# chacorp/latent-nerf-test

Hardware: AMD Instinct MI355X
Metric: latent-frames/sec (64x64x4, 128^3 grid), render forward+backward (higher is better)
Workload: dtype bf16

## Files before the change

### latent-nerf-test_amd/csrc/mlp_bf16.hip

```cpp
#include "common.h"
#include "mlp_shared.h"

namespace lnerf {

typedef __bf16 bf16x8 __attribute__((ext_vector_type(8)));
#define MFMA32(a, b, c) __builtin_amdgcn_mfma_f32_16x16x32_bf16((a), (b), (c), 0, 0, 0)

constexpr int F_W1A = 0;
constexpr int F_W2A = 4;
constexpr int F_W3A = 12;
constexpr int F_W3T = 14;
constexpr int F_W2T = 18;
constexpr int F_W1T = 26;
constexpr int F_FWD = 14, F_ALL = 30;

constexpr int RS = 68;

__device__ __forceinline__ int phi_of(int s, int q, int jj) { return 32 * s + 16 * (jj >> 2) + 4 * q + (jj & 3); }

__device__ __forceinline__ int frag_source(int e, int out_dim, int &idx) {
    const int f = e >> 9, l = (e >> 3) & 63, jj = e & 7;
    const int q = l >> 4, c = l & 15;
    if (f < F_W2A) {
        idx = (16 * (f - F_W1A) + c) * MLP_IN + 8 * q + jj;
        return 1;
    } else if (f < F_W3A) {
        const int mt = (f - F_W2A) >> 1, s = (f - F_W2A) & 1;
        idx = (16 * mt + c) * MLP_HID + phi_of(s, q, jj);
        return 2;
    } else if (f < F_W3T) {
        const int s = f - F_W3A;
        idx = c * MLP_HID + phi_of(s, q, jj);
        return c < out_dim ? 3 : 0;
    } else if (f < F_W2T) {
        const int mt = f - F_W3T, n = 4 * q + jj;
        idx = n * MLP_HID + 16 * mt + c;
        return (jj < 4 && n < out_dim) ? 3 : 0;
    } else if (f < F_W1T) {
        const int mt = (f - F_W2T) >> 1, s = (f - F_W2T) & 1;
        idx = phi_of(s, q, jj) * MLP_HID + 16 * mt + c;
        return 2;
    }
    const int mt = (f - F_W1T) >> 1, s = (f - F_W1T) & 1;
    idx = phi_of(s, q, jj) * MLP_IN + 16 * mt + c;
    return 1;
}

__device__ __forceinline__ void build_fragments(const MlpArgs &a, __bf16 *frag, int n_frag, int tid, int nthreads) {
    for (int e = tid; e < n_frag * 512; e += nthreads) {
        int idx;
        const int t = frag_source(e, a.out_dim, idx);
        const float v = t == 1 ? a.w1[idx] : t == 2 ? a.w2[idx] : t == 3 ? a.w3[idx] : 0.f;
        frag[e] = (__bf16)v;
    }
}

__global__ void __launch_bounds__(256) k_mlp_fragment_maps(int out_dim, int32_t *m1, int32_t *m2, int32_t *m3) {
    for (int e = blockIdx.x * 256 + threadIdx.x; e < F_ALL * 512; e += gridDim.x * 256) {
        int idx;
        const int t = frag_source(e, out_dim, idx);
        const int slot = (e >> 9) < F_W3T ? 0 : 1;
        int32_t *m = t == 1 ? m1 : t == 2 ? m2 : t == 3 ? m3 : nullptr;
        if (m) m[2 * idx + slot] = e;
    }
}

constexpr int F_SELX = 30;
constexpr int F_SEL3 = 32;
constexpr int F_SW = 33;
static_assert((size_t)F_SW * 1024 <= MLP_FRAG_BYTES, "fragment cache");
__device__ __forceinline__ void build_selectors(__bf16 *frag, int tid, int nthreads) {
    for (int e = tid; e < (F_SW - F_SELX) * 512; e += nthreads) {
        const int f = F_SELX + (e >> 9), l = (e >> 3) & 63, jj = e & 7;
        const int q = l >> 4, c = l & 15;
        const bool one = f < F_SEL3 ? (8 * q + jj == 16 * (f - F_SELX) + c) : (jj < 4 && 4 * q + jj == c);
        frag[F_SELX * 512 + e] = (__bf16)(one ? 1.0f : 0.0f);
    }
}
__global__ void __launch_bounds__(256) k_mlp_build_fragments(MlpArgs a, __bf16 *out, int n_frag) {
    build_fragments(a, out, n_frag < F_ALL ? n_frag : F_ALL, blockIdx.x * 256 + threadIdx.x, gridDim.x * 256);
    if (n_frag > F_ALL) build_selectors(out, blockIdx.x * 256 + threadIdx.x, gridDim.x * 256);
}
__device__ __forceinline__ void fetch_fragments(const MlpArgs &a, __bf16 *frag, int n_frag, int tid, int nthreads) {
    if (a.frag_global) {
        const uint4 *src = reinterpret_cast<const uint4 *>(a.frag_global);
        uint4 *dst = reinterpret_cast<uint4 *>(frag);
        for (int e = tid; e < n_frag * 64; e += nthreads) dst[e] = src[e];
    } else {
        build_fragments(a, frag, n_frag, tid, nthreads);
    }
}

__device__ __forceinline__ bf16x8 ld_frag(const __bf16 *frag, int f, int lane) {
    return *reinterpret_cast<const bf16x8 *>(frag + (f * 64 + lane) * 8);
}

__device__ __forceinline__ bf16x8 load_x(const MlpArgs &a, int64_t m, int q) {
    if (a.feat_bf16) {
        const char *f = reinterpret_cast<const char *>(a.feat);
        const uint32_t ls = (uint32_t)a.level_stride;
        uint32_t w[4];
#pragma unroll
        for (int k = 0; k < 4; ++k)
            w[k] = *reinterpret_cast<const uint32_t *>(f + (size_t)((((uint32_t)(4 * q + k)) * ls + (uint32_t)m) << 2));
        return *reinterpret_cast<bf16x8 *>(w);
    }
    bf16x8 x;
    const float2 *f = reinterpret_cast<const float2 *>(a.feat);
#pragma unroll
    for (int k = 0; k < 4; ++k) {
        const float2 v = f[(int64_t)(4 * q + k) * a.level_stride + m];
        x[2 * k] = (__bf16)v.x;
        x[2 * k + 1] = (__bf16)v.y;
    }
    return x;
}
__device__ __forceinline__ int64_t clamp_row(int64_t m, int64_t M) { return m < M ? m : (M > 0 ? M - 1 : 0); }

typedef short s16x2 __attribute__((ext_vector_type(2)));
typedef unsigned short u16x2 __attribute__((ext_vector_type(2)));
typedef __bf16 bf16x2 __attribute__((ext_vector_type(2)));

__device__ __forceinline__ uint32_t cvt_pk(float lo, float hi) {
    typedef float f32x2 __attribute__((ext_vector_type(2)));
    const f32x2 f = {lo, hi};
    return __builtin_bit_cast(uint32_t, __builtin_convertvector(f, bf16x2));
}
__device__ __forceinline__ uint32_t relu_pk(uint32_t v) {
    const s16x2 z = {0, 0};
    return __builtin_bit_cast(uint32_t, __builtin_elementwise_max(__builtin_bit_cast(s16x2, v), z));
}
__device__ __forceinline__ uint32_t live_pk(uint32_t act) {
    asm("" : "+v"(act));
    const s16x2 z = {0, 0};
    const s16x2 n = z - __builtin_bit_cast(s16x2, act);
    return __builtin_bit_cast(uint32_t, n >> 15);
}
union Pk8 {
    bf16x8 v;
    uint32_t u[4];
};
__device__ __forceinline__ bf16x8 pack_relu_pk(const f32x4 &lo, const f32x4 &hi) {
    Pk8 r;
    r.u[0] = relu_pk(cvt_pk(lo[0], lo[1]));
    r.u[1] = relu_pk(cvt_pk(lo[2], lo[3]));
    r.u[2] = relu_pk(cvt_pk(hi[0], hi[1]));
    r.u[3] = relu_pk(cvt_pk(hi[2], hi[3]));
    return r.v;
}
__device__ __forceinline__ bf16x8 pack_masked_pk(const f32x4 &lo, const f32x4 &hi, const bf16x8 &act) {
    Pk8 r, a;
    a.v = act;
    r.u[0] = cvt_pk(lo[0], lo[1]) & live_pk(a.u[0]);
    r.u[1] = cvt_pk(lo[2], lo[3]) & live_pk(a.u[1]);
    r.u[2] = cvt_pk(hi[0], hi[1]) & live_pk(a.u[2]);
    r.u[3] = cvt_pk(hi[2], hi[3]) & live_pk(a.u[3]);
    return r.v;
}
__device__ __forceinline__ bf16x8 pack_plain_pk(const f32x4 &lo, const f32x4 &hi) {
    Pk8 r;
    r.u[0] = cvt_pk(lo[0], lo[1]);
    r.u[1] = cvt_pk(lo[2], lo[3]);
    r.u[2] = cvt_pk(hi[0], hi[1]);
    r.u[3] = cvt_pk(hi[2], hi[3]);
    return r.v;
}
__device__ __forceinline__ float sum8(const bf16x8 &v, float acc) {
    Pk8 a;
    a.v = v;
    bf16x2 ones;
    ones[0] = (__bf16)1.0f;
    ones[1] = (__bf16)1.0f;
#pragma unroll
    for (int i = 0; i < 4; ++i) acc = __builtin_amdgcn_fdot2_f32_bf16(__builtin_bit_cast(bf16x2, a.u[i]), ones, acc, false);
    return acc;
}

__device__ __forceinline__ bf16x8 pack_relu(const f32x4 &lo, const f32x4 &hi) { return pack_relu_pk(lo, hi); }
__device__ __forceinline__ bf16x8 pack_masked(const f32x4 &lo, const f32x4 &hi, const bf16x8 &act) {
    return pack_masked_pk(lo, hi, act);
}

__device__ __forceinline__ f32x4 ld_bias4(const float *b, int base) {
    return (f32x4){b[base], b[base + 1], b[base + 2], b[base + 3]};
}

#ifdef LNERF_STAMPS
__device__ unsigned long long g_mlp_stamps[32];
struct Stamps {
    unsigned long long acc[16], prev;
    __device__ __forceinline__ void init() {
        for (int i = 0; i < 16; ++i) acc[i] = 0;
        prev = __builtin_amdgcn_s_memtime();
    }
    __device__ __forceinline__ void mark(int k) {
        const unsigned long long now = __builtin_amdgcn_s_memtime();
        acc[k] += now - prev;
        prev = now;
    }
    __device__ __forceinline__ void flush(int base) {
        if (threadIdx.x == 0)
            for (int i = 0; i < 16; ++i) atomicAdd(&g_mlp_stamps[base + i], acc[i]);
    }
};
#else
struct Stamps {
    __device__ __forceinline__ void init() {}
    __device__ __forceinline__ void mark(int) {}
    __device__ __forceinline__ void flush(int) {}
};
#endif

template <int T>
__device__ __forceinline__ void forward_hidden(const __bf16 *frag, const float *sB1, const float *sB2, int lane,
                                               const bf16x8 xB[T], bf16x8 h1B[2][T], bf16x8 h2B[2][T], Stamps &st) {
    const int q = lane >> 4;
    f32x4 acc[4][T];
#pragma unroll
    for (int mt = 0; mt < 4; ++mt) {
        const bf16x8 w = ld_frag(frag, F_W1A + mt, lane);
        const f32x4 b = ld_bias4(sB1, 16 * mt + 4 * q);
#pragma unroll
        for (int t = 0; t < T; ++t) acc[mt][t] = MFMA32(w, xB[t], b);
    }
#pragma unroll
    for (int s = 0; s < 2; ++s)
#pragma unroll
        for (int t = 0; t < T; ++t) h1B[s][t] = pack_relu(acc[2 * s][t], acc[2 * s + 1][t]);
    st.mark(1);
#pragma unroll
    for (int mt = 0; mt < 4; ++mt) {
        const f32x4 b = ld_bias4(sB2, 16 * mt + 4 * q);
#pragma unroll
        for (int t = 0; t < T; ++t) acc[mt][t] = b;
#pragma unroll
        for (int s = 0; s < 2; ++s) {
            const bf16x8 w = ld_frag(frag, F_W2A + 2 * mt + s, lane);
#pragma unroll
            for (int t = 0; t < T; ++t) acc[mt][t] = MFMA32(w, h1B[s][t], acc[mt][t]);
        }
    }
#pragma unroll
    for (int s = 0; s < 2; ++s)
#pragma unroll
        for (int t = 0; t < T; ++t) h2B[s][t] = pack_relu(acc[2 * s][t], acc[2 * s + 1][t]);
    st.mark(2);
}

template <int WPS>
__global__ void __launch_bounds__(256, WPS)
k_mlp_forward_bf16(MlpArgs a, float *__restrict__ sigmas, float *__restrict__ rgbs) {
    __shared__ __attribute__((aligned(16))) __bf16 frag[F_FWD * 512];
    __shared__ float sB1[MLP_HID], sB2[MLP_HID], sB3[16];
    int64_t M = a.m_host;
    if (a.m_dev) { const int64_t md = *a.m_dev; M = md < M ? md : M; }
    const int tid = threadIdx.x, lane = tid & 63, w = tid >> 6, q = lane >> 4, c = lane & 15;
    fetch_fragments(a, frag, F_FWD, tid, 256);
    if (tid < MLP_HID) { sB1[tid] = a.b1[tid]; sB2[tid] = a.b2[tid]; }
    if (tid < 16) sB3[tid] = tid < a.out_dim ? a.b3[tid] : 0.f;
    __syncthreads();
    const int nrgb = a.out_dim - 1;
    bf16x8 xB[2];
#pragma unroll
    for (int t = 0; t < 2; ++t) {
        const int64_t m = (int64_t)blockIdx.x * 128 + w * 32 + 16 * t + c;
        xB[t] = load_x(a, clamp_row(m, M), q);
    }
    Stamps st;
    st.init();
    for (int64_t tile = blockIdx.x; tile * 128 < M; tile += gridDim.x) {
        const int64_t m0 = tile * 128 + w * 32;
        bf16x8 xB_n[2], h1B[2][2], h2B[2][2];
#pragma unroll
        for (int t = 0; t < 2; ++t) {
            const int64_t m = m0 + (int64_t)gridDim.x * 128 + 16 * t + c;
            xB_n[t] = load_x(a, clamp_row(m, M), q);
        }
        st.mark(0);
        forward_hidden<2>(frag, sB1, sB2, lane, xB, h1B, h2B, st);
        const f32x4 b3 = ld_bias4(sB3, 4 * q);
        int lane3 = lane;
        asm("" : "+v"(lane3) : "s"((int)tile));
        const bf16x8 w3a = ld_frag(frag, F_W3A, lane3), w3b = ld_frag(frag, F_W3A + 1, lane3);
#pragma unroll
        for (int t = 0; t < 2; ++t) {
            f32x4 o = b3;
            o = MFMA32(w3a, h2B[0][t], o);
            o = MFMA32(w3b, h2B[1][t], o);
            const int64_t m = m0 + 16 * t + c;
            if (a.out_dim == 5) {
                const float r3 = __shfl_down(o[0], 16, 64);
                if (q == 0 && m < M) {
                    sigmas[m] = expf(o[0] + blob_of(a, m));
                    reinterpret_cast<float4 *>(rgbs)[m] = make_float4(o[1], o[2], o[3], r3);
                }
            } else if (m < M) {
#pragma unroll
                for (int r = 0; r < 4; ++r) {
                    const int n = 4 * q + r;
                    if (n == 0) sigmas[m] = expf(o[r] + blob_of(a, m));
                    else if (n < a.out_dim) rgbs[m * nrgb + (n - 1)] = o[r];
                }
            }
        }
        st.mark(3);
        xB[0] = xB_n[0];
        xB[1] = xB_n[1];
    }
    st.flush(0);
}

template <int T>
struct Upstream { float v[T][4], sg[T]; };

template <int T>
__device__ __forceinline__ Upstream<T> load_upstream(const MlpArgs &a, const float *__restrict__ sigmas,
                                                     const float *__restrict__ dsigmas, const float *__restrict__ drgbs,
                                                     int64_t m0, int64_t M, int q, int c) {
    const int nrgb = a.out_dim - 1;
    Upstream<T> u;
#pragma unroll
    for (int t = 0; t < T; ++t) {
        const int64_t m = m0 + 16 * t + c;
        const bool in = m < M;
        const int64_t mc = clamp_row(m, M);
        if (a.out_dim == 5) {
            const float ds = dsigmas[mc], sg = sigmas[mc];
            const float4 g = reinterpret_cast<const float4 *>(drgbs)[mc];
            const bool q0 = in && q == 0, q1 = in && q == 1;
            u.sg[t] = sg;
            u.v[t][0] = q0 ? ds : (q1 ? g.w : 0.f);
            u.v[t][1] = q0 ? g.x : 0.f;
            u.v[t][2] = q0 ? g.y : 0.f;
            u.v[t][3] = q0 ? g.z : 0.f;
        } else {
            u.sg[t] = 1.0f;
#pragma unroll
            for (int jj = 0; jj < 4; ++jj) u.v[t][jj] = 0.f;
            if (in && q == 0) { u.v[t][0] = dsigmas[m]; u.sg[t] = sigmas[m]; }
#pragma unroll
            for (int jj = 0; jj < 4; ++jj) {
                const int n = 4 * q + jj;
                if (in && n >= 1 && n < a.out_dim) u.v[t][jj] = drgbs[m * nrgb + (n - 1)];
            }
        }
    }
    return u;
}
__device__ __forceinline__ bool upstream_fragment(const float v[4], float sg, int q, bf16x8 &d3) {
    const float e15 = 3269017.3724721107f;
    const float v0 = q == 0 ? v[0] * fminf(sg, e15) : v[0];
    Pk8 d;
    d.u[0] = cvt_pk(v0, v[1]);
    d.u[1] = cvt_pk(v[2], v[3]);
    d.u[2] = 0u;
    d.u[3] = 0u;
    d3 = d.v;
    return (v0 != 0.f) || (v[1] != 0.f) || (v[2] != 0.f) || (v[3] != 0.f);
}

__device__ __forceinline__ void stage_pair(__bf16 *img, int row, int fa, int fb, const bf16x8 &v) {
    const uint4 u = *reinterpret_cast<const uint4 *>(&v);
    *reinterpret_cast<uint2 *>(img + row * RS + fa) = make_uint2(u.x, u.y);
    *reinterpret_cast<uint2 *>(img + row * RS + fb) = make_uint2(u.z, u.w);
}
__device__ __forceinline__ void stage_lo(__bf16 *img, int row, int fa, const bf16x8 &v) {
    const uint4 u = *reinterpret_cast<const uint4 *>(&v);
    *reinterpret_cast<uint2 *>(img + row * RS + fa) = make_uint2(u.x, u.y);
}

typedef short s16x4 __attribute__((ext_vector_type(4)));
__device__ __forceinline__ bf16x8 ld_tr(const __bf16 *img, int k, int f0, int lane) {
    typedef s16x4 __attribute__((address_space(3))) *lds_s16x4_p;
    const int g = lane >> 4, i = lane & 15;
    const __bf16 *p = img + (32 * k + 8 * g + (i >> 2)) * RS + f0 + 4 * (i & 3);
    union {
        struct { s16x4 lo, hi; } h;
        bf16x8 v;
    } u;
    u.h.lo = __builtin_amdgcn_ds_read_tr16_b64_v4i16((lds_s16x4_p)p);
    u.h.hi = __builtin_amdgcn_ds_read_tr16_b64_v4i16((lds_s16x4_p)(p + 4 * RS));
    return u.v;
}

template <int NW, int T>
__global__ void __launch_bounds__(NW * 64, (NW == 4 ? 2 : 4))
k_mlp_backward_bf16(MlpArgs a, const float *__restrict__ sigmas, const float *__restrict__ dsigmas,
                    const float *__restrict__ drgbs, float *__restrict__ dfeat, float *__restrict__ slabs) {
    constexpr int STEP = NW * 16 * T, KS = STEP / 32, NH = NW / 4, C2 = 4 / NH, C1 = 2 / NH;
    __shared__ __attribute__((aligned(16))) __bf16 frag[F_ALL * 512];
    __shared__ __attribute__((aligned(16))) __bf16 imgA[STEP * RS];
    __shared__ __attribute__((aligned(16))) __bf16 imgD[STEP * RS];
    __shared__ float sB1[MLP_HID], sB2[MLP_HID];
    int64_t M = a.m_host;
    if (a.m_dev) { const int64_t md = *a.m_dev; M = md < M ? md : M; }
    const int tid = threadIdx.x, lane = tid & 63, w = tid >> 6, q = lane >> 4, c = lane & 15;
    const int r = w & 3, h = w >> 2;
    fetch_fragments(a, frag, F_ALL, tid, NW * 64);
    if (tid < MLP_HID) { sB1[tid] = a.b1[tid]; sB2[tid] = a.b2[tid]; }
    __syncthreads();
    const f32x4 zero4 = (f32x4){0.f, 0.f, 0.f, 0.f};
    bf16x8 ones;
#pragma unroll
    for (int i = 0; i < 8; ++i) ones[i] = (__bf16)1.0f;

    f32x4 gW2[C2], gW1[C1], gB = zero4, gW3 = zero4;
    f32x4 gB1x = zero4, gB3 = zero4;
#pragma unroll
    for (int i = 0; i < C2; ++i) gW2[i] = zero4;
#pragma unroll
    for (int i = 0; i < C1; ++i) gW1[i] = zero4;
    const bool own_b2 = h == 0, own_b1 = h == NH - 1, own_w3 = h == 0, own_b3 = w == NW - 4;

    const int64_t wofs = (int64_t)w * 16 * T;
    Upstream<T> up = load_upstream<T>(a, sigmas, dsigmas, drgbs, (int64_t)blockIdx.x * STEP + wofs, M, q, c);
    bf16x8 xB[T];
#pragma unroll
    for (int t = 0; t < T; ++t) {
        const int64_t m = (int64_t)blockIdx.x * STEP + wofs + 16 * t + c;
        xB[t] = load_x(a, clamp_row(m, M), q);
    }
    Stamps st;
    st.init();
    for (int64_t tile = blockIdx.x; tile * STEP < M; tile += gridDim.x) {
        const int64_t m0 = tile * STEP + wofs, m1 = m0 + (int64_t)gridDim.x * STEP;
        const Upstream<T> up_c = up;
        bf16x8 xC[T], h1B[2][T], h2B[2][T], dzB[2][T], d3B[T];
#pragma unroll
        for (int t = 0; t < T; ++t) xC[t] = xB[t];
        up = load_upstream<T>(a, sigmas, dsigmas, drgbs, m1, M, q, c);
#pragma unroll
        for (int t = 0; t < T; ++t) xB[t] = load_x(a, clamp_row(m1 + 16 * t + c, M), q);
        bool live = false;
#pragma unroll
        for (int t = 0; t < T; ++t) live = upstream_fragment(up_c.v[t], up_c.sg[t], q, d3B[t]) || live;
        (void)live;
        st.mark(4);
        forward_hidden<T>(frag, sB1, sB2, lane, xC, h1B, h2B, st);
        __syncthreads();
        st.mark(5);
#pragma unroll
        for (int t = 0; t < T; ++t) {
            const int row = 16 * T * w + 16 * t + c;
#pragma unroll
            for (int s = 0; s < 2; ++s) stage_pair(imgA, row, 32 * s + 4 * q, 32 * s + 16 + 4 * q, h2B[s][t]);
            stage_lo(imgD, row, 4 * q, d3B[t]);
        }
        __syncthreads();
        st.mark(6);
        if (own_w3 || own_b3) {
#pragma unroll
            for (int k = 0; k < KS; ++k) {
                const bf16x8 dA = ld_tr(imgD, k, 0, lane);
                if (own_w3) gW3 = MFMA32(dA, ld_tr(imgA, k, 16 * r, lane), gW3);
                if (own_b3) gB3 = MFMA32(dA, ones, gB3);
            }
        }
        st.mark(7);
        {
            f32x4 acc[4][T];
#pragma unroll
            for (int mt = 0; mt < 4; ++mt) {
                const bf16x8 wf = ld_frag(frag, F_W3T + mt, lane);
#pragma unroll
                for (int t = 0; t < T; ++t) acc[mt][t] = MFMA32(wf, d3B[t], zero4);
            }
#pragma unroll
            for (int s = 0; s < 2; ++s)
#pragma unroll
                for (int t = 0; t < T; ++t) dzB[s][t] = pack_masked(acc[2 * s][t], acc[2 * s + 1][t], h2B[s][t]);
        }
        st.mark(8);
        __syncthreads();
#pragma unroll
        for (int t = 0; t < T; ++t) {
            const int row = 16 * T * w + 16 * t + c;
#pragma unroll
            for (int s = 0; s < 2; ++s) {
                stage_pair(imgA, row, 32 * s + 4 * q, 32 * s + 16 + 4 * q, h1B[s][t]);
                stage_pair(imgD, row, 32 * s + 4 * q, 32 * s + 16 + 4 * q, dzB[s][t]);
            }
        }
        __syncthreads();
        st.mark(9);
#pragma unroll
        for (int k = 0; k < KS; ++k) {
            const bf16x8 dA = ld_tr(imgD, k, 16 * r, lane);
#pragma unroll
            for (int i = 0; i < C2; ++i) gW2[i] = MFMA32(dA, ld_tr(imgA, k, 16 * (C2 * h + i), lane), gW2[i]);
            if (own_b2) gB = MFMA32(dA, ones, gB);
        }
        st.mark(10);
        {
            f32x4 acc[4][T];
#pragma unroll
            for (int mt = 0; mt < 4; ++mt) {
#pragma unroll
                for (int t = 0; t < T; ++t) acc[mt][t] = zero4;
#pragma unroll
                for (int s = 0; s < 2; ++s) {
                    const bf16x8 wf = ld_frag(frag, F_W2T + 2 * mt + s, lane);
#pragma unroll
                    for (int t = 0; t < T; ++t) acc[mt][t] = MFMA32(wf, dzB[s][t], acc[mt][t]);
                }
            }
#pragma unroll
            for (int s = 0; s < 2; ++s)
#pragma unroll
                for (int t = 0; t < T; ++t) dzB[s][t] = pack_masked(acc[2 * s][t], acc[2 * s + 1][t], h1B[s][t]);
        }
        st.mark(11);
        __syncthreads();
#pragma unroll
        for (int t = 0; t < T; ++t) {
            const int row = 16 * T * w + 16 * t + c;
            stage_pair(imgA, row, 8 * q, 8 * q + 4, xC[t]);
#pragma unroll
            for (int s = 0; s < 2; ++s) stage_pair(imgD, row, 32 * s + 4 * q, 32 * s + 16 + 4 * q, dzB[s][t]);
        }
        __syncthreads();
        st.mark(12);
#pragma unroll
        for (int k = 0; k < KS; ++k) {
            const bf16x8 dA = ld_tr(imgD, k, 16 * r, lane);
#pragma unroll
            for (int i = 0; i < C1; ++i) gW1[i] = MFMA32(dA, ld_tr(imgA, k, 16 * (C1 * h + i), lane), gW1[i]);
            if (own_b1) { if (NH == 1) gB1x = MFMA32(dA, ones, gB1x); else gB = MFMA32(dA, ones, gB); }
        }
        st.mark(13);
#pragma unroll
        for (int mt = 0; mt < 2; ++mt) {
            f32x4 ax[T];
#pragma unroll
            for (int t = 0; t < T; ++t) ax[t] = zero4;
#pragma unroll
            for (int s = 0; s < 2; ++s) {
                const bf16x8 wf = ld_frag(frag, F_W1T + 2 * mt + s, lane);
#pragma unroll
                for (int t = 0; t < T; ++t) ax[t] = MFMA32(wf, dzB[s][t], ax[t]);
            }
#pragma unroll
            for (int t = 0; t < T; ++t) {
                const int64_t m = m0 + 16 * t + c;
                if (m < M) {
                    const int lv = 8 * mt + 2 * q;
                    char *df = reinterpret_cast<char *>(dfeat);
                    const uint32_t ls = (uint32_t)a.level_stride, o0 = (((uint32_t)lv) * ls + (uint32_t)m) << 3;
                    *reinterpret_cast<float2 *>(df + (size_t)o0) = make_float2(ax[t][0], ax[t][1]);
                    *reinterpret_cast<float2 *>(df + (size_t)(o0 + (ls << 3))) = make_float2(ax[t][2], ax[t][3]);
                }
            }
        }
        st.mark(14);
    }

    st.flush(16);
    float *slab = slabs + (int64_t)blockIdx.x * MLP_SLAB;
#pragma unroll
    for (int rr = 0; rr < 4; ++rr) {
        const int o = 16 * r + 4 * q + rr;
#pragma unroll
        for (int i = 0; i < C2; ++i) slab[MLP_SL_W2 + o * MLP_HID + 16 * (C2 * h + i) + c] = gW2[i][rr];
#pragma unroll
        for (int i = 0; i < C1; ++i) slab[MLP_SL_W1 + o * MLP_IN + 16 * (C1 * h + i) + c] = gW1[i][rr];
        if (c == 0) {
            if (own_b2) slab[MLP_SL_B2 + o] = gB[rr];
            if (own_b1) slab[MLP_SL_B1 + o] = NH == 1 ? gB1x[rr] : gB[rr];
        }
        if (own_w3) slab[MLP_SL_W3 + (4 * q + rr) * MLP_HID + 16 * r + c] = gW3[rr];
        if (own_b3 && c == 0) slab[MLP_SL_B3 + 4 * q + rr] = gB3[rr];
    }
}

}

namespace lnerf {

#ifdef LNERF_STAMPS
int mlp_stamps_read(unsigned long long *out32) {
    unsigned long long z[32] = {0};
    if (hipMemcpyFromSymbol(out32, HIP_SYMBOL(g_mlp_stamps), sizeof(z)) != hipSuccess) return LNERF_ERR_HIP;
    if (hipMemcpyToSymbol(HIP_SYMBOL(g_mlp_stamps), z, sizeof(z)) != hipSuccess) return LNERF_ERR_HIP;
    return LNERF_OK;
}
#endif

int launch_mlp_fragment_maps(int out_dim, int32_t *m1, int32_t *m2, int32_t *m3, hipStream_t stream) {
    if (hipMemsetAsync(m1, 0xFF, (size_t)MLP_HID * MLP_IN * 2 * sizeof(int32_t), stream) != hipSuccess ||
        hipMemsetAsync(m2, 0xFF, (size_t)MLP_HID * MLP_HID * 2 * sizeof(int32_t), stream) != hipSuccess ||
        hipMemsetAsync(m3, 0xFF, (size_t)out_dim * MLP_HID * 2 * sizeof(int32_t), stream) != hipSuccess) {
        set_error("mlp_fragment_maps: hipMemsetAsync failed");
        return LNERF_ERR_HIP;
    }
    hipLaunchKernelGGL(k_mlp_fragment_maps, dim3(16), dim3(256), 0, stream, out_dim, m1, m2, m3);
    LNERF_CHECK_LAUNCH("mlp(fragment maps)");
    return LNERF_OK;
}

int launch_mlp_fragments_bf16(const MlpArgs &a, void *frag_out, bool backward_too, hipStream_t stream) {
    const int n = backward_too ? F_SW : F_FWD;
    hipLaunchKernelGGL(k_mlp_build_fragments, dim3((unsigned)(n * 2)), dim3(256), 0, stream, a, (__bf16 *)frag_out, n);
    LNERF_CHECK_LAUNCH("mlp(fragments)");
    return LNERF_OK;
}

int launch_mlp_forward_bf16(const MlpArgs &a, float *sigmas, float *rgbs, int blocks, int wps, hipStream_t stream) {
    if (wps >= 3) hipLaunchKernelGGL(k_mlp_forward_bf16<3>, dim3((unsigned)blocks), dim3(256), 0, stream, a, sigmas, rgbs);
    else hipLaunchKernelGGL(k_mlp_forward_bf16<2>, dim3((unsigned)blocks), dim3(256), 0, stream, a, sigmas, rgbs);
    LNERF_CHECK_LAUNCH("mlp_forward(bf16)");
    return LNERF_OK;
}

int launch_mlp_backward_bf16(const MlpArgs &a, const float *sigmas, const float *dsigmas, const float *drgbs,
                             float *dfeat, float *slabs, int blocks, hipStream_t stream) {
    hipLaunchKernelGGL((k_mlp_backward_bf16<4, 2>), dim3((unsigned)blocks), dim3(256), 0, stream, a, sigmas, dsigmas,
                       drgbs, dfeat, slabs);
    LNERF_CHECK_LAUNCH("mlp_backward(bf16)");
    return LNERF_OK;
}

}
```

### latent-nerf-test_amd/csrc/mlp_shared.h

```cpp
#pragma once
#include "common.h"

namespace lnerf {

typedef float f32x4 __attribute__((ext_vector_type(4)));

constexpr int MLP_IN = 32, MLP_HID = 64, MLP_OUTP = 16;

constexpr int MLP_SL_W1 = 0, MLP_SL_B1 = MLP_SL_W1 + MLP_HID * MLP_IN, MLP_SL_W2 = MLP_SL_B1 + MLP_HID,
              MLP_SL_B2 = MLP_SL_W2 + MLP_HID * MLP_HID, MLP_SL_W3 = MLP_SL_B2 + MLP_HID,
              MLP_SL_B3 = MLP_SL_W3 + MLP_OUTP * MLP_HID, MLP_SLAB = MLP_SL_B3 + MLP_OUTP;
constexpr int MLP_BWD_MAX_BLOCKS = 512;

struct MlpArgs {
    const void *feat;
    int feat_bf16;
    int64_t level_stride;
    const float *xyzs;
    const float *w1, *b1, *w2, *b2, *w3, *b3;
    int out_dim;
    float blob_scale, blob_denom;
    int64_t m_host;
    const int32_t *m_dev;
    const void *frag_global;
};
constexpr size_t MLP_FRAG_BYTES = LNERF_MLP_FRAGMENT_BYTES;

__device__ __forceinline__ float blob_of(const MlpArgs &a, int64_t m) {
    const float x = a.xyzs[m * 3], y = a.xyzs[m * 3 + 1], z = a.xyzs[m * 3 + 2];
    const float d2 = (x * x + y * y) + z * z;
    return a.blob_scale * expf(-d2 / a.blob_denom);
}

int launch_mlp_fragments_bf16(const MlpArgs &a, void *frag_out, bool backward_too, hipStream_t stream);
int launch_mlp_fragment_maps(int out_dim, int32_t *m1, int32_t *m2, int32_t *m3, hipStream_t stream);
int launch_mlp_forward_bf16(const MlpArgs &a, float *sigmas, float *rgbs, int blocks, int wps, hipStream_t stream);
int launch_mlp_backward_bf16(const MlpArgs &a, const float *sigmas, const float *dsigmas, const float *drgbs,
                             float *dfeat, float *slabs, int blocks, hipStream_t stream);

#ifdef LNERF_STAMPS
int mlp_stamps_read(unsigned long long *out32);
#endif

}
```

Baseline: 2663.

## Specialize MLP kernels on feature dtype/output width, prefetch positions, hold weights in registers

The forward and backward MLP kernels are now templated on whether features are bf16 and whether out_dim is 5, so runtime branches disappear. The forward kernel keeps the W1/W2 fragments and b1 bias in registers across tiles instead of re-reading them from LDS each tile. It also software-prefetches xyz positions for the blob term together with the next tile's features. Empty asm pins and sched_barriers force the prefetched loads to stay in flight across the compute, at the cost of higher VGPR pressure, which may reduce occupancy or cause spills.

```diff
diff --git a/latent-nerf-test_amd/csrc/mlp_bf16.hip b/latent-nerf-test_amd/csrc/mlp_bf16.hip
--- a/latent-nerf-test_amd/csrc/mlp_bf16.hip
+++ b/latent-nerf-test_amd/csrc/mlp_bf16.hip
@@ -95,8 +95,9 @@
     return *reinterpret_cast<const bf16x8 *>(frag + (f * 64 + lane) * 8);
 }
 
+template <bool FB16>
 __device__ __forceinline__ bf16x8 load_x(const MlpArgs &a, int64_t m, int q) {
-    if (a.feat_bf16) {
+    if (FB16) {
         const char *f = reinterpret_cast<const char *>(a.feat);
         const uint32_t ls = (uint32_t)a.level_stride;
         uint32_t w[4];
@@ -211,15 +212,30 @@
 };
 #endif
 
+struct HeldFragments {
+    bf16x8 w1[4], w2[8];
+    f32x4 b1[4];
+    __device__ __forceinline__ void read(const __bf16 *frag, const float *sB1, int lane) {
+#pragma unroll
+        for (int mt = 0; mt < 4; ++mt) {
+            w1[mt] = ld_frag(frag, F_W1A + mt, lane);
+            b1[mt] = ld_bias4(sB1, 16 * mt + 4 * (lane >> 4));
+        }
+#pragma unroll
+        for (int i = 0; i < 8; ++i) w2[i] = ld_frag(frag, F_W2A + i, lane);
+    }
+};
+
 template <int T>
 __device__ __forceinline__ void forward_hidden(const __bf16 *frag, const float *sB1, const float *sB2, int lane,
-                                               const bf16x8 xB[T], bf16x8 h1B[2][T], bf16x8 h2B[2][T], Stamps &st) {
+                                               const bf16x8 xB[T], bf16x8 h1B[2][T], bf16x8 h2B[2][T], Stamps &st,
+                                               const HeldFragments *held = nullptr) {
     const int q = lane >> 4;
     f32x4 acc[4][T];
 #pragma unroll
     for (int mt = 0; mt < 4; ++mt) {
-        const bf16x8 w = ld_frag(frag, F_W1A + mt, lane);
-        const f32x4 b = ld_bias4(sB1, 16 * mt + 4 * q);
+        const bf16x8 w = held ? held->w1[mt] : ld_frag(frag, F_W1A + mt, lane);
+        const f32x4 b = held ? held->b1[mt] : ld_bias4(sB1, 16 * mt + 4 * q);
 #pragma unroll
         for (int t = 0; t < T; ++t) acc[mt][t] = MFMA32(w, xB[t], b);
     }
@@ -235,7 +251,7 @@
         for (int t = 0; t < T; ++t) acc[mt][t] = b;
 #pragma unroll
         for (int s = 0; s < 2; ++s) {
-            const bf16x8 w = ld_frag(frag, F_W2A + 2 * mt + s, lane);
+            const bf16x8 w = held ? held->w2[2 * mt + s] : ld_frag(frag, F_W2A + 2 * mt + s, lane);
 #pragma unroll
             for (int t = 0; t < T; ++t) acc[mt][t] = MFMA32(w, h1B[s][t], acc[mt][t]);
         }
@@ -247,7 +263,15 @@
     st.mark(2);
 }
 
-template <int WPS>
+typedef uint32_t u32x4 __attribute__((ext_vector_type(4)));
+__device__ __forceinline__ void pin_x(bf16x8 &a, bf16x8 &b) {
+    u32x4 ua = __builtin_bit_cast(u32x4, a), ub = __builtin_bit_cast(u32x4, b);
+    asm volatile("" : "+v"(ua), "+v"(ub));
+    a = __builtin_bit_cast(bf16x8, ua);
+    b = __builtin_bit_cast(bf16x8, ub);
+}
+
+template <int WPS, bool FB16, bool OUT5>
 __global__ void __launch_bounds__(256, WPS)
 k_mlp_forward_bf16(MlpArgs a, float *__restrict__ sigmas, float *__restrict__ rgbs) {
     __shared__ __attribute__((aligned(16))) __bf16 frag[F_FWD * 512];
@@ -261,45 +285,61 @@
     __syncthreads();
     const int nrgb = a.out_dim - 1;
     bf16x8 xB[2];
+    Pos3 pos[2];
 #pragma unroll
     for (int t = 0; t < 2; ++t) {
-        const int64_t m = (int64_t)blockIdx.x * 128 + w * 32 + 16 * t + c;
-        xB[t] = load_x(a, clamp_row(m, M), q);
-    }
+        const int64_t mc = clamp_row((int64_t)blockIdx.x * 128 + w * 32 + 16 * t + c, M);
+        xB[t] = load_x<FB16>(a, mc, q);
+        pos[t] = load_pos(a, mc);
+    }
+    pin_x(xB[0], xB[1]);
+    asm volatile("" : "+v"(pos[0].x), "+v"(pos[0].y), "+v"(pos[0].z), "+v"(pos[1].x), "+v"(pos[1].y), "+v"(pos[1].z));
+    HeldFragments held;
+    held.read(frag, sB1, lane);
     Stamps st;
     st.init();
     for (int64_t tile = blockIdx.x; tile * 128 < M; tile += gridDim.x) {
         const int64_t m0 = tile * 128 + w * 32;
+        float blob[2];
+#pragma unroll
+        for (int t = 0; t < 2; ++t) blob[t] = blob_at(a, pos[t]);
         bf16x8 xB_n[2], h1B[2][2], h2B[2][2];
 #pragma unroll
         for (int t = 0; t < 2; ++t) {
-            const int64_t m = m0 + (int64_t)gridDim.x * 128 + 16 * t + c;
-            xB_n[t] = load_x(a, clamp_row(m, M), q);
-        }
+            const int64_t mc = clamp_row(m0 + (int64_t)gridDim.x * 128 + 16 * t + c, M);
+            xB_n[t] = load_x<FB16>(a, mc, q);
+            pos[t] = load_pos(a, mc);
+        }
+        __builtin_amdgcn_sched_barrier(0);
         st.mark(0);
-        forward_hidden<2>(frag, sB1, sB2, lane, xB, h1B, h2B, st);
+        forward_hidden<2>(frag, sB1, sB2, lane, xB, h1B, h2B, st, &held);
         const f32x4 b3 = ld_bias4(sB3, 4 * q);
-        int lane3 = lane;
-        asm("" : "+v"(lane3) : "s"((int)tile));
-        const bf16x8 w3a = ld_frag(frag, F_W3A, lane3), w3b = ld_frag(frag, F_W3A + 1, lane3);
+        const bf16x8 w3a = ld_frag(frag, F_W3A, lane), w3b = ld_frag(frag, F_W3A + 1, lane);
+        f32x4 o[2];
 #pragma unroll
         for (int t = 0; t < 2; ++t) {
-            f32x4 o = b3;
-            o = MFMA32(w3a, h2B[0][t], o);
-            o = MFMA32(w3b, h2B[1][t], o);
+            o[t] = MFMA32(w3a, h2B[0][t], b3);
+            o[t] = MFMA32(w3b, h2B[1][t], o[t]);
+        }
+        __builtin_amdgcn_sched_barrier(0);
+        pin_x(xB_n[0], xB_n[1]);
+        asm volatile("" : "+v"(pos[0].x), "+v"(pos[0].y), "+v"(pos[0].z), "+v"(pos[1].x), "+v"(pos[1].y), "+v"(pos[1].z),
+                          "+v"(o[0]), "+v"(o[1]));
+#pragma unroll
+        for (int t = 0; t < 2; ++t) {
             const int64_t m = m0 + 16 * t + c;
-            if (a.out_dim == 5) {
-                const float r3 = __shfl_down(o[0], 16, 64);
+            if (OUT5) {
+                const float r3 = __shfl_down(o[t][0], 16, 64);
                 if (q == 0 && m < M) {
-                    sigmas[m] = expf(o[0] + blob_of(a, m));
-                    reinterpret_cast<float4 *>(rgbs)[m] = make_float4(o[1], o[2], o[3], r3);
+                    sigmas[m] = expf(o[t][0] + blob[t]);
+                    reinterpret_cast<float4 *>(rgbs)[m] = make_float4(o[t][1], o[t][2], o[t][3], r3);
                 }
             } else if (m < M) {
 #pragma unroll
                 for (int r = 0; r < 4; ++r) {
                     const int n = 4 * q + r;
-                    if (n == 0) sigmas[m] = expf(o[r] + blob_of(a, m));
-                    else if (n < a.out_dim) rgbs[m * nrgb + (n - 1)] = o[r];
+                    if (n == 0) sigmas[m] = expf(o[t][r] + blob[t]);
+                    else if (n < a.out_dim) rgbs[m * nrgb + (n - 1)] = o[t][r];
                 }
             }
         }
@@ -310,44 +350,46 @@
     st.flush(0);
 }
 
+template <int T, bool OUT5>
+struct Upstream;
 template <int T>
-struct Upstream { float v[T][4], sg[T]; };
-
+struct Upstream<T, true> { f32x4 g[T]; float ds[T], sg[T]; };
 template <int T>
-__device__ __forceinline__ Upstream<T> load_upstream(const MlpArgs &a, const float *__restrict__ sigmas,
-                                                     const float *__restrict__ dsigmas, const float *__restrict__ drgbs,
-                                                     int64_t m0, int64_t M, int q, int c) {
+struct Upstream<T, false> { float v[T][4], sg[T]; };
+
+template <int T>
+__device__ __forceinline__ void load_upstream(Upstream<T, true> &u, const MlpArgs &a, const float *__restrict__ sigmas,
+                                              const float *__restrict__ dsigmas, const float *__restrict__ drgbs,
+                                              int64_t m0, int64_t M, int q, int c) {
+#pragma unroll
+    for (int t = 0; t < T; ++t) {
+        const int64_t mc = clamp_row(m0 + 16 * t + c, M);
+        u.ds[t] = dsigmas[mc];
+        u.sg[t] = sigmas[mc];
+        u.g[t] = reinterpret_cast<const f32x4 *>(drgbs)[mc];
+    }
+}
+template <int T>
+__device__ __forceinline__ void load_upstream(Upstream<T, false> &u, const MlpArgs &a, const float *__restrict__ sigmas,
+                                              const float *__restrict__ dsigmas, const float *__restrict__ drgbs,
+                                              int64_t m0, int64_t M, int q, int c) {
     const int nrgb = a.out_dim - 1;
-    Upstream<T> u;
 #pragma unroll
     for (int t = 0; t < T; ++t) {
         const int64_t m = m0 + 16 * t + c;
         const bool in = m < M;
-        const int64_t mc = clamp_row(m, M);
-        if (a.out_dim == 5) {
-            const float ds = dsigmas[mc], sg = sigmas[mc];
-            const float4 g = reinterpret_cast<const float4 *>(drgbs)[mc];
-            const bool q0 = in && q == 0, q1 = in && q == 1;
-            u.sg[t] = sg;
-            u.v[t][0] = q0 ? ds : (q1 ? g.w : 0.f);
-            u.v[t][1] = q0 ? g.x : 0.f;
-            u.v[t][2] = q0 ? g.y : 0.f;
-            u.v[t][3] = q0 ? g.z : 0.f;
-        } else {
-            u.sg[t] = 1.0f;
-#pragma unroll
-            for (int jj = 0; jj < 4; ++jj) u.v[t][jj] = 0.f;
-            if (in && q == 0) { u.v[t][0] = dsigmas[m]; u.sg[t] = sigmas[m]; }
-#pragma unroll
-            for (int jj = 0; jj < 4; ++jj) {
-                const int n = 4 * q + jj;
-                if (in && n >= 1 && n < a.out_dim) u.v[t][jj] = drgbs[m * nrgb + (n - 1)];
-            }
-        }
-    }
-    return u;
-}
-__device__ __forceinline__ bool upstream_fragment(const float v[4], float sg, int q, bf16x8 &d3) {
+        u.sg[t] = 1.0f;
+#pragma unroll
+        for (int jj = 0; jj < 4; ++jj) u.v[t][jj] = 0.f;
+        if (in && q == 0) { u.v[t][0] = dsigmas[m]; u.sg[t] = sigmas[m]; }
+#pragma unroll
+        for (int jj = 0; jj < 4; ++jj) {
+            const int n = 4 * q + jj;
+            if (in && n >= 1 && n < a.out_dim) u.v[t][jj] = drgbs[m * nrgb + (n - 1)];
+        }
+    }
+}
+__device__ __forceinline__ void upstream_fragment(const float v[4], float sg, int q, bf16x8 &d3) {
     const float e15 = 3269017.3724721107f;
     const float v0 = q == 0 ? v[0] * fminf(sg, e15) : v[0];
     Pk8 d;
@@ -356,7 +398,32 @@
     d.u[2] = 0u;
     d.u[3] = 0u;
     d3 = d.v;
-    return (v0 != 0.f) || (v[1] != 0.f) || (v[2] != 0.f) || (v[3] != 0.f);
+}
+template <int T>
+__device__ __forceinline__ void upstream_fragment(const Upstream<T, true> &u, int t, bool in, int q, bf16x8 &d3) {
+    const bool q0 = in && q == 0, q1 = in && q == 1;
+    const float v[4] = {q0 ? u.ds[t] : (q1 ? u.g[t][3] : 0.f), q0 ? u.g[t][0] : 0.f, q0 ? u.g[t][1] : 0.f,
+                        q0 ? u.g[t][2] : 0.f};
+    upstream_fragment(v, u.sg[t], q, d3);
+}
+template <int T>
+__device__ __forceinline__ void upstream_fragment(const Upstream<T, false> &u, int t, bool, int q, bf16x8 &d3) {
+    upstream_fragment(u.v[t], u.sg[t], q, d3);
+}
+__device__ __forceinline__ void pin_step(bf16x8 x[2], Upstream<2, true> &u, f32x4 ax[2][2]) {
+    u32x4 x0 = __builtin_bit_cast(u32x4, x[0]), x1 = __builtin_bit_cast(u32x4, x[1]);
+    asm volatile("" : "+v"(x0), "+v"(x1), "+v"(u.g[0]), "+v"(u.g[1]), "+v"(u.ds[0]), "+v"(u.ds[1]), "+v"(u.sg[0]),
+                      "+v"(u.sg[1]), "+v"(ax[0][0]), "+v"(ax[0][1]), "+v"(ax[1][0]), "+v"(ax[1][1]));
+    x[0] = __builtin_bit_cast(bf16x8, x0);
+    x[1] = __builtin_bit_cast(bf16x8, x1);
+}
+__device__ __forceinline__ void pin_step(bf16x8 x[2], Upstream<2, false> &u, f32x4 ax[2][2]) {
+    u32x4 x0 = __builtin_bit_cast(u32x4, x[0]), x1 = __builtin_bit_cast(u32x4, x[1]);
+    asm volatile("" : "+v"(x0), "+v"(x1), "+v"(u.v[0][0]), "+v"(u.v[0][1]), "+v"(u.v[0][2]), "+v"(u.v[0][3]),
+                      "+v"(u.v[1][0]), "+v"(u.v[1][1]), "+v"(u.v[1][2]), "+v"(u.v[1][3]), "+v"(u.sg[0]), "+v"(u.sg[1]),
+                      "+v"(ax[0][0]), "+v"(ax[0][1]), "+v"(ax[1][0]), "+v"(ax[1][1]));
+    x[0] = __builtin_bit_cast(bf16x8, x0);
+    x[1] = __builtin_bit_cast(bf16x8, x1);
 }
 
 __device__ __forceinline__ void stage_pair(__bf16 *img, int row, int fa, int fb, const bf16x8 &v) {
@@ -383,7 +450,7 @@
     return u.v;
 }
 
-template <int NW, int T>
+template <int NW, int T, bool FB16, bool OUT5>
 __global__ void __launch_bounds__(NW * 64, (NW == 4 ? 2 : 4))
 k_mlp_backward_bf16(MlpArgs a, const float *__restrict__ sigmas, const float *__restrict__ dsigmas,
                     const float *__restrict__ drgbs, float *__restrict__ dfeat, float *__restrict__ slabs) {
@@ -412,29 +479,33 @@
     for (int i = 0; i < C1; ++i) gW1[i] = zero4;
     const bool own_b2 = h == 0, own_b1 = h == NH - 1, own_w3 = h == 0, own_b3 = w == NW - 4;
 
+    static_assert(T == 2, "pin_step");
     const int64_t wofs = (int64_t)w * 16 * T;
-    Upstream<T> up = load_upstream<T>(a, sigmas, dsigmas, drgbs, (int64_t)blockIdx.x * STEP + wofs, M, q, c);
+    Upstream<T, OUT5> up;
+    load_upstream<T>(up, a, sigmas, dsigmas, drgbs, (int64_t)blockIdx.x * STEP + wofs, M, q, c);
     bf16x8 xB[T];
 #pragma unroll
     for (int t = 0; t < T; ++t) {
         const int64_t m = (int64_t)blockIdx.x * STEP + wofs + 16 * t + c;
-        xB[t] = load_x(a, clamp_row(m, M), q);
+        xB[t] = load_x<FB16>(a, clamp_row(m, M), q);
+    }
+    {
+        f32x4 none[2][T] = {{zero4, zero4}, {zero4, zero4}};
+        pin_step(xB, up, none);
     }
     Stamps st;
     st.init();
     for (int64_t tile = blockIdx.x; tile * STEP < M; tile += gridDim.x) {
         const int64_t m0 = tile * STEP + wofs, m1 = m0 + (int64_t)gridDim.x * STEP;
-        const Upstream<T> up_c = up;
+        const Upstream<T, OUT5> up_c = up;
         bf16x8 xC[T], h1B[2][T], h2B[2][T], dzB[2][T], d3B[T];
 #pragma unroll
         for (int t = 0; t < T; ++t) xC[t] = xB[t];
-        up = load_upstream<T>(a, sigmas, dsigmas, drgbs, m1, M, q, c);
-#pragma unroll
-        for (int t = 0; t < T; ++t) xB[t] = load_x(a, clamp_row(m1 + 16 * t + c, M), q);
-        bool live = false;
-#pragma unroll
-        for (int t = 0; t < T; ++t) live = upstream_fragment(up_c.v[t], up_c.sg[t], q, d3B[t]) || live;
-        (void)live;
+        load_upstream<T>(up, a, sigmas, dsigmas, drgbs, m1, M, q, c);
+#pragma unroll
+        for (int t = 0; t < T; ++t) xB[t] = load_x<FB16>(a, clamp_row(m1 + 16 * t + c, M), q);
+#pragma unroll
+        for (int t = 0; t < T; ++t) upstream_fragment<T>(up_c, t, m0 + 16 * t + c < M, q, d3B[t]);
         st.mark(4);
         forward_hidden<T>(frag, sB1, sB2, lane, xC, h1B, h2B, st);
         __syncthreads();
@@ -528,17 +599,22 @@
             if (own_b1) { if (NH == 1) gB1x = MFMA32(dA, ones, gB1x); else gB = MFMA32(dA, ones, gB); }
         }
         st.mark(13);
+        f32x4 ax[2][T];
 #pragma unroll
         for (int mt = 0; mt < 2; ++mt) {
-            f32x4 ax[T];
-#pragma unroll
-            for (int t = 0; t < T; ++t) ax[t] = zero4;
+#pragma unroll
+            for (int t = 0; t < T; ++t) ax[mt][t] = zero4;
 #pragma unroll
             for (int s = 0; s < 2; ++s) {
                 const bf16x8 wf = ld_frag(frag, F_W1T + 2 * mt + s, lane);
 #pragma unroll
-                for (int t = 0; t < T; ++t) ax[t] = MFMA32(wf, dzB[s][t], ax[t]);
+                for (int t = 0; t < T; ++t) ax[mt][t] = MFMA32(wf, dzB[s][t], ax[mt][t]);
             }
+        }
+        __builtin_amdgcn_sched_barrier(0);
+        pin_step(xB, up, ax);
+#pragma unroll
+        for (int mt = 0; mt < 2; ++mt) {
 #pragma unroll
             for (int t = 0; t < T; ++t) {
                 const int64_t m = m0 + 16 * t + c;
@@ -546,8 +622,8 @@
                     const int lv = 8 * mt + 2 * q;
                     char *df = reinterpret_cast<char *>(dfeat);
                     const uint32_t ls = (uint32_t)a.level_stride, o0 = (((uint32_t)lv) * ls + (uint32_t)m) << 3;
-                    *reinterpret_cast<float2 *>(df + (size_t)o0) = make_float2(ax[t][0], ax[t][1]);
-                    *reinterpret_cast<float2 *>(df + (size_t)(o0 + (ls << 3))) = make_float2(ax[t][2], ax[t][3]);
+                    *reinterpret_cast<float2 *>(df + (size_t)o0) = make_float2(ax[mt][t][0], ax[mt][t][1]);
+                    *reinterpret_cast<float2 *>(df + (size_t)(o0 + (ls << 3))) = make_float2(ax[mt][t][2], ax[mt][t][3]);
                 }
             }
         }
@@ -604,17 +680,38 @@
     return LNERF_OK;
 }
 
+template <int WPS>
+static void launch_forward_wps(const MlpArgs &a, float *sigmas, float *rgbs, int blocks, hipStream_t stream) {
+    const dim3 g((unsigned)blocks), b(256);
+    if (a.feat_bf16) {
+        if (a.out_dim == 5) hipLaunchKernelGGL((k_mlp_forward_bf16<WPS, true, true>), g, b, 0, stream, a, sigmas, rgbs);
+        else hipLaunchKernelGGL((k_mlp_forward_bf16<WPS, true, false>), g, b, 0, stream, a, sigmas, rgbs);
+    } else {
+        if (a.out_dim == 5) hipLaunchKernelGGL((k_mlp_forward_bf16<WPS, false, true>), g, b, 0, stream, a, sigmas, rgbs);
+        else hipLaunchKernelGGL((k_mlp_forward_bf16<WPS, false, false>), g, b, 0, stream, a, sigmas, rgbs);
+    }
+}
 int launch_mlp_forward_bf16(const MlpArgs &a, float *sigmas, float *rgbs, int blocks, int wps, hipStream_t stream) {
-    if (wps >= 3) hipLaunchKernelGGL(k_mlp_forward_bf16<3>, dim3((unsigned)blocks), dim3(256), 0, stream, a, sigmas, rgbs);
-    else hipLaunchKernelGGL(k_mlp_forward_bf16<2>, dim3((unsigned)blocks), dim3(256), 0, stream, a, sigmas, rgbs);
+    if (wps >= 3) launch_forward_wps<3>(a, sigmas, rgbs, blocks, stream);
+    else launch_forward_wps<2>(a, sigmas, rgbs, blocks, stream);
     LNERF_CHECK_LAUNCH("mlp_forward(bf16)");
     return LNERF_OK;
 }
 
 int launch_mlp_backward_bf16(const MlpArgs &a, const float *sigmas, const float *dsigmas, const float *drgbs,
                              float *dfeat, float *slabs, int blocks, hipStream_t stream) {
-    hipLaunchKernelGGL((k_mlp_backward_bf16<4, 2>), dim3((unsigned)blocks), dim3(256), 0, stream, a, sigmas, dsigmas,
-                       drgbs, dfeat, slabs);
+    const dim3 g((unsigned)blocks), b(256);
+    if (a.feat_bf16) {
+        if (a.out_dim == 5)
+            hipLaunchKernelGGL((k_mlp_backward_bf16<4, 2, true, true>), g, b, 0, stream, a, sigmas, dsigmas, drgbs, dfeat, slabs);
+        else
+            hipLaunchKernelGGL((k_mlp_backward_bf16<4, 2, true, false>), g, b, 0, stream, a, sigmas, dsigmas, drgbs, dfeat, slabs);
+    } else {
+        if (a.out_dim == 5)
+            hipLaunchKernelGGL((k_mlp_backward_bf16<4, 2, false, true>), g, b, 0, stream, a, sigmas, dsigmas, drgbs, dfeat, slabs);
+        else
+            hipLaunchKernelGGL((k_mlp_backward_bf16<4, 2, false, false>), g, b, 0, stream, a, sigmas, dsigmas, drgbs, dfeat, slabs);
+    }
     LNERF_CHECK_LAUNCH("mlp_backward(bf16)");
     return LNERF_OK;
 }
diff --git a/latent-nerf-test_amd/csrc/mlp_shared.h b/latent-nerf-test_amd/csrc/mlp_shared.h
--- a/latent-nerf-test_amd/csrc/mlp_shared.h
+++ b/latent-nerf-test_amd/csrc/mlp_shared.h
@@ -26,11 +26,15 @@
 };
 constexpr size_t MLP_FRAG_BYTES = LNERF_MLP_FRAGMENT_BYTES;
 
-__device__ __forceinline__ float blob_of(const MlpArgs &a, int64_t m) {
-    const float x = a.xyzs[m * 3], y = a.xyzs[m * 3 + 1], z = a.xyzs[m * 3 + 2];
-    const float d2 = (x * x + y * y) + z * z;
+struct Pos3 { float x, y, z; };
+__device__ __forceinline__ Pos3 load_pos(const MlpArgs &a, int64_t m) {
+    return Pos3{a.xyzs[m * 3], a.xyzs[m * 3 + 1], a.xyzs[m * 3 + 2]};
+}
+__device__ __forceinline__ float blob_at(const MlpArgs &a, const Pos3 &p) {
+    const float d2 = (p.x * p.x + p.y * p.y) + p.z * p.z;
     return a.blob_scale * expf(-d2 / a.blob_denom);
 }
+__device__ __forceinline__ float blob_of(const MlpArgs &a, int64_t m) { return blob_at(a, load_pos(a, m)); }
 
 int launch_mlp_fragments_bf16(const MlpArgs &a, void *frag_out, bool backward_too, hipStream_t stream);
 int launch_mlp_fragment_maps(int out_dim, int32_t *m1, int32_t *m2, int32_t *m3, hipStream_t stream);
```

Result: faster. 2717 (median of 6 runs) (+2.0%).
